# intelligent-machine-learning/tfplus

Hardware: AMD Instinct MI355X
Metric: lookups+GroupAdam-applies/sec and HBM GB/s, 1M int64 ids x dim32 (higher is better)
Workload: dtype f32; 1 GPU; configs[1]: 50M-key KvVariable x dim32 per GPU, 1000000 ids/batch per GPU Zipf(1.2), lookup + sparse GroupAdam apply; keys=50000000, dim=32, batch=1000000, global_batch=1000000, parallelism=single GPU

## Files before the change

tfplus_amd/csrc/kv_device.h:

```cpp
#pragma once

constexpr long long EMPTY_KEY = (long long)0x8000000000000000ULL;
constexpr unsigned FLAG_BLACK = 1u;
constexpr unsigned FLAG_UNDER = 2u;
constexpr unsigned FLAG_DIRTY = 4u;
constexpr float CUTOFF = 1.0e-20f;
constexpr unsigned FLAG_FREE = 8u;
constexpr unsigned ROW_TOMB = 0xFFFFFFFFu;
constexpr unsigned ROW_FILTERED = 0x80000000u;
constexpr unsigned ROW_MASK = 0x7FFFFFFFu;
constexpr unsigned HEAD_BIT = 0x80000000u;
constexpr unsigned BASE_MASK = 0x3FFFFFFFu;
constexpr int RANK_SHIFT = 21;
constexpr unsigned SLOT_MASK = (1u << RANK_SHIFT) - 1u;
constexpr int LCOLD = 16;
constexpr int HC = 128;
constexpr unsigned EP_TAG = 0x40000000u;
constexpr unsigned NEW_BIT = 0x80000000u;
constexpr unsigned HINT_NEW = 0xFFFFFFFFu;
constexpr int HC2 = 512;

constexpr int TB = 256;
#ifndef KV_TBT
#define KV_TBT 512
// ... 198 lines not shown
  return r;
}

__device__ __forceinline__ void init_rule_rows(const TableDev& t, long long key, const float** ia, const float** ib, int D) {
  const unsigned long long h = pick64((unsigned long long)key ^ (t.seed * 0x9E3779B97F4A7C15ULL));
  *ia = t.init_table + (size_t)((unsigned)h % t.init_rows) * D;
  *ib = t.init_table + (size_t)((unsigned)(h >> 32) % t.init_rows) * D;
}
__device__ __forceinline__ void init_rule_rows(const TableDev& t, long long key, const float** ia, const float** ib) {
  init_rule_rows(t, key, ia, ib, t.dim);
}
__device__ __forceinline__ bool init_row_coop(const TableDev& t, long long key, float* dst,
                                              int lane, int lanes) {
  const float *a, *b;
  init_rule_rows(t, key, &a, &b);
  bool big = false;
  for (int e = lane; e < t.dim; e += lanes) {
    float v = (a[e] + b[e]) * 0.5f;
    dst[e] = v;
    big |= fabsf(v) >= CUTOFF;
  }
  return big;
}

__device__ __forceinline__ unsigned part_of(long long key, int pshift) {
  return pshift >= 64 ? 0u : (unsigned)(mix64((unsigned long long)key) >> pshift);
}

__device__ __forceinline__ void lds_barrier() { asm volatile("s_waitcnt lgkmcnt(0)\n\ts_barrier" ::: "memory"); }

template <int NW, bool LDSONLY = false>
__device__ __forceinline__ unsigned block_excl_scan(unsigned v, unsigned* wtot, unsigned* total) {
  const int lane = threadIdx.x & 63, wv = threadIdx.x >> 6;
  unsigned incl = v;
#pragma unroll
  for (int o = 1; o < 64; o <<= 1) {
    const unsigned x = __shfl_up(incl, o);
    if (lane >= o) incl += x;
  }
  if (LDSONLY) lds_barrier(); else __syncthreads();
  if (lane == 63) wtot[wv] = incl;
  if (LDSONLY) lds_barrier(); else __syncthreads();
  unsigned base = 0, tot = 0;
#pragma unroll
  for (int i = 0; i < NW; ++i) {
    const unsigned x = wtot[i];
    if (i < wv) base += x;
    tot += x;
  }
  *total = tot;
  return base + incl - v;
}

template <typename IdT>
__device__ __forceinline__ long long load_id(const IdT* ids, size_t i) {
  return (long long)ids[i];
}
struct IdCount { long long id, count; };
template <>
__device__ __forceinline__ long long load_id<IdCount>(const IdCount* ids, size_t i) { return ids[i].id; }

#ifdef KV_FASTM_CONST
#define KV_FASTM(a) (KV_FASTM_CONST != 0)
#else
#define KV_FASTM(a) ((a).fast != 0)
#endif
__device__ __forceinline__ float kv_sqrt(float x, bool fast) { return fast ? __builtin_amdgcn_sqrtf(x) : sqrtf(x); }
__device__ __forceinline__ float kv_div(float x, float y, bool fast) { return fast ? x * __builtin_amdgcn_rcpf(y) : x / y; }

__device__ __forceinline__ unsigned slot_find_or_insert(const TableDev& t, long long key,
                                                       unsigned day, bool* inserted) {
  unsigned r = table_find_or_insert(t, key, inserted);
  if (r == 0) return 0;
  unsigned* fp = freq_ptr(t, r);
  if (*inserted) {
    *fp = 1u;
  } else {
    unsigned lo = (*fp & 0xFFFFu) + 1u;
    if (lo > 65535u) lo = 65535u;
    *fp = (day << 16) | lo;
  }
  return r;
}

template <int V>
__device__ __forceinline__ void ldv(const float* p, float (&o)[V]) {
  if (V == 4) {
    const float4 t4 = *reinterpret_cast<const float4*>(p);
    o[0] = t4.x; o[1 % V] = t4.y; o[2 % V] = t4.z; o[3 % V] = t4.w;
  } else {
    o[0] = p[0];
  }
}
template <int V>
__device__ __forceinline__ void ldv_stream(const float* p, float (&o)[V]) {
#pragma unroll
  for (int c = 0; c < V; ++c) o[c] = __builtin_nontemporal_load(p + c);
}
template <int V>
__device__ __forceinline__ void stv(float* p, const float (&o)[V]) {
  if (V == 4) {
    *reinterpret_cast<float4*>(p) = make_float4(o[0], o[1 % V], o[2 % V], o[3 % V]);
  } else {
    p[0] = o[0];
  }
}
// ... 461 lines not shown
```

tfplus_amd/csrc/kv_fused.h:

```cpp
#pragma once

__device__ __forceinline__ unsigned tile_insert(const TableDev& t, long long key) {
  Entry* slot;
  unsigned long long stored;
  unsigned long long p = 0;
  const bool sentinel = key == EMPTY_KEY;
  if (sentinel) { slot = &t.entries[t.mask + 1]; stored = 0ull; }
  else { stored = (unsigned long long)key; p = mix64((unsigned long long)key) & t.mask; slot = &t.entries[p]; }
  for (;;) {
    const Entry e = load_entry(slot);
    if ((unsigned long long)e.key == stored && !(sentinel && e.key == EMPTY_KEY)) {
      if (e.row == ROW_TOMB) {
        if (atomicCAS(&slot->row, ROW_TOMB, 0u) == ROW_TOMB) break;
        return NEW_BIT;
      }
      if (e.row == 0u || e.hint == HINT_NEW) return NEW_BIT | e.row;
      return e.row;
    }
    if (e.key == EMPTY_KEY) {
      const unsigned long long old = atomicCAS(reinterpret_cast<unsigned long long*>(&slot->key),
                                               (unsigned long long)EMPTY_KEY, stored);
      if (old == (unsigned long long)EMPTY_KEY) break;
      if (old == stored) return NEW_BIT;
      if (sentinel) continue;
// ... 406 lines not shown
      unsigned before = 0;
      for (int wv = 0; wv < TBT / 64; ++wv) {
        if (wave == wv && valid) {
          before = run[e];
          if (rw == 0u) run[e] = (unsigned short)(before + cnt);
        }
        lds_barrier();
      }
      myrank[k] = valid ? before + rw : 0u;
    }
  }
#pragma unroll
  for (int k = 0; k < IPT; ++k) {
    if (tslot[k] == 0xFFFFFFFFu || sm.lcnt[tslot[k]] <= 1u) continue;
    const unsigned pre = sm.escan[sm.lpos[tslot[k]]];
    sm.mr[(pre & ES_POS) + myrank[k]] = (unsigned)(k * TBT + tid) | ((pre >> ES_NSH) << 11) | (myrank[k] == 0u ? 0x80000000u : 0u);
  }
  if (has_counts) {
    lds_barrier();
    for (unsigned e = tid; e <= (unsigned)TILE; e += TBT) sm.hist[e] = 0;
    lds_barrier();
#pragma unroll
    for (int k = 0; k < IPT; ++k)
      if (tslot[k] != 0xFFFFFFFFu) atomicAdd(&sm.hist[sm.lpos[tslot[k]]], creg[k]);
    lds_barrier();
#pragma unroll
    for (int k = 0; k < IPT; ++k) {
      if (wpos[k] == 0xFFFFFFFFu) continue;
      const unsigned f = sm.hist[wpos[k]];
      w.ent_a[(size_t)tile * TILE + wpos[k]] = wcnt[k] | ((f > 65535u ? 65535u : f) << 16);
    }
  }
  lds_barrier();
  {
    unsigned* dst = w.mrow + (size_t)tile * TILE;
    for (int j = tid; j < TILE; j += TBT) dst[j] = sm.mr[j];
  }
  KV_STAMP(4);
  if constexpr (GATHER) {
#pragma unroll
    for (int k = 0; k < IPT; ++k) rr[k] = tslot[k] != 0xFFFFFFFFu ? sm.lrow[tslot[k]] : 0u;
    if (__builtin_expect(pf == 1.2345678e-38f, 0)) sm.wtot[0] = 1u;
    output_rows();
  }
  KV_STAMP(5);
}

template <typename IdT, int VQ, bool GATHER, bool NOTABLE = false>
__global__ void __launch_bounds__(TBT, 4) k_ltile(TableDev t, WsDev w, const IdT* __restrict__ ids,
                                              const int* __restrict__ counts, long long n, int det, float* __restrict__ out) {
  ltile_body<IdT, VQ, GATHER, NOTABLE>(t, w, ids, counts, n, det, out);
}

template <int T, int NW>
__device__ __forceinline__ unsigned seg_directory_t(const WsDev& w, unsigned p, unsigned short* tpre,
                                                    unsigned short* tstart, unsigned* wtot, unsigned* pbase) {
  const unsigned NT = w.ntiles;
  unsigned run0 = 0, pb = 0;
  for (unsigned tb = 0; tb < NT; tb += T) {
    const unsigned t = tb + threadIdx.x;
    unsigned len = 0, s0 = 0;
    if (t < NT) {
      const unsigned* c0 = w.toff + (size_t)t * (w.P + 1) + p;
      const unsigned a = c0[0], b = c0[1];
      s0 = a & 0xFFFFu;
      len = (b & 0xFFFFu) - s0;
      tstart[t] = (unsigned short)s0;
    }
    unsigned tot;
    const unsigned ex = block_excl_scan<NW>(len, wtot, &tot);
    unsigned tot2;
    block_excl_scan<NW>(s0, wtot, &tot2);
    if (t < NT) tpre[t] = (unsigned short)min(run0 + ex, 65535u);
    run0 += tot;
    pb += tot2;
  }
  __syncthreads();
  *pbase = pb;
  return run0;
}
__device__ __forceinline__ void part2_body(const WsDev& w, const PartArgs& a) {
  constexpr int HSK = 1024;
  constexpr int UCAPK = HSK - TBK;
  constexpr int EB = 8;
  __shared__ long long hkey[HSK + 1];
  __shared__ unsigned hval[HSK + 1];
  __shared__ unsigned hrow[HSK + 1];
  __shared__ unsigned short lnew[UCAPK + 8];
  __shared__ unsigned short ulist[UCAPK + 8];
  __shared__ unsigned lnu, lsent, lnnew, lkeys;
  __shared__ unsigned wtot[8];
  extern __shared__ __attribute__((aligned(16))) char smem_raw[];
  unsigned short* tpre = reinterpret_cast<unsigned short*>(smem_raw);
  unsigned short* tstart = tpre + w.ntiles;

  const int tid = threadIdx.x;
  const unsigned p = xcd_partition(blockIdx.x, w.P);
  const unsigned NT = w.ntiles;
  const int D = a.tv.dim;
  KV_STAMPP(0);
  unsigned pbase;
  const unsigned E = seg_directory_t<TBK, TBK / 64>(w, p, tpre, tstart, wtot, &pbase);
  if (E == 0) return;
  __shared__ unsigned stkR[24], stkr[24];
  __shared__ int sp;
  if (tid == 0) { stkR[0] = 1; stkr[0] = 0; sp = 1; lkeys = 0; }
  __syncthreads();
  if (E > 65535u) {
    if (tid == 0) raise_error(a.tv, 2u);
    return;
  }
  while (sp > 0) {
    const unsigned R = stkR[sp - 1], round = stkr[sp - 1];
    __syncthreads();
    if (tid == 0) --sp;
    for (int s = tid; s <= HSK; s += TBK) { hkey[s] = EMPTY_KEY; hval[s] = 0; hrow[s] = 0; }
    if (tid == 0) { lnu = 0; lsent = 0; lnnew = 0; }
    __syncthreads();
    for (unsigned x0 = 0; x0 < E; x0 += EB * TBK) {
      unsigned ge[EB];
      long long key[EB];
      unsigned ea[EB], rw[EB];
#pragma unroll
      for (int k = 0; k < EB; ++k) {
        const unsigned x = x0 + k * TBK + tid;
        ge[k] = x < E ? (unsigned)seg_entry(tpre, tstart, NT, x) : 0xFFFFFFFFu;
      }
#pragma unroll
      for (int k = 0; k < EB; ++k) {
        key[k] = 0; ea[k] = 0; rw[k] = 0;
        if (ge[k] != 0xFFFFFFFFu) { key[k] = w.ent_key[ge[k]]; ea[k] = w.ent_a[ge[k]]; rw[k] = w.ent_b[ge[k]]; }
      }
#pragma unroll
      for (int k = 0; k < EB; ++k) {
        if (ge[k] == 0xFFFFFFFFu || !in_round(key[k], R, round)) continue;
        if (lnu >= (unsigned)UCAPK) continue;
        bool first;
        const unsigned h = lds_key_slot<HSK>(hkey, &lsent, key[k], true, &first);
        if (first) {
          const unsigned u = atomicAdd(&lnu, 1u);
          if (u < (unsigned)UCAPK) ulist[u] = (unsigned short)h;
        }
        atomicAdd(&hval[h], ea[k] >> 16);
        atomicMax(&hrow[h], rw[k]);
      }
    }
    __syncthreads();
    if (lnu >= (unsigned)UCAPK) {
      __syncthreads();
      if (tid == 0) {
        if (sp + 2 <= 24) {
          stkR[sp] = 2 * R; stkr[sp] = round; ++sp;
          stkR[sp] = 2 * R; stkr[sp] = round + R; ++sp;
        } else {
          raise_error(a.tv, 2u);
        }
      }
      __syncthreads();
      continue;
    }
    KV_STAMPP(1);
    const unsigned nu = lnu;
    if (tid == 0) lkeys += nu;

    constexpr int PERU = (UCAPK + TBK - 1) / TBK;
    {
      unsigned sl[PERU], r[PERU];
      bool isnew[PERU];
      uint2 m[PERU];
#pragma unroll
      for (int k = 0; k < PERU; ++k) {
        const unsigned u = tid * PERU + k;
        sl[k] = 0xFFFFFFFFu; r[k] = 0; isnew[k] = false; m[k] = make_uint2(0u, (unsigned)FLAG_DIRTY);
        if (u < nu) {
          sl[k] = ulist[u];
          const unsigned rw = hrow[sl[k]];
          r[k] = rw & ROW_MASK; isnew[k] = (rw & NEW_BIT) != 0u;
          if (r[k] != 0u && !isnew[k]) m[k] = load_freq_flags(a.tv, r[k]);
        }
      }
#pragma unroll
      for (int k = 0; k < PERU; ++k) {
        if (sl[k] == 0xFFFFFFFFu) continue;
        const unsigned s = sl[k];
        const long long key = (s == HSK) ? EMPTY_KEY : hkey[s];
        if (__builtin_expect(isnew[k], 0)) {
          Entry* e = table_entry_of(a.tv, key);
          if (e) {
            if (r[k] == 0u) { const unsigned er = load_entry(e).row; r[k] = er != ROW_TOMB ? er : 0u; }
            e->hint = 0u;
          }
          hrow[s] = r[k] | NEW_BIT;
        }
        if (r[k] == 0u) continue;
        RowMeta* mp = meta_ptr(a.tv, r[k]);
        if (isnew[k]) { mp->key = key; mp->delta = 0; mp->stamp = 0; }
        mark_delta(a.tv, r[k]);
        const unsigned cnt = a.count_once ? 1u : hval[s];
        mp->freq = (a.day << 16) | freq_add_sat(m[k].x, cnt);
        if (isnew[k]) mp->flags = (unsigned char)FLAG_DIRTY;
        if (m[k].y & FLAG_DIRTY) lnew[atomicAdd(&lnnew, 1u)] = (unsigned short)(s | (isnew[k] ? 0x8000u : 0u));
      }
    }
    __syncthreads();
    KV_STAMPP(2);

    {
      const int lane8 = tid & 7;
      const unsigned nn = lnnew;
      const unsigned npad = (nn + 7u) & ~7u;
      for (unsigned j = tid >> 3; j < npad; j += TBK / 8) {
        const bool live = j < nn;
        const unsigned sv = live ? lnew[j] : 0u;
        const unsigned s = sv & 0x7FFFu;
        const bool isnew = (sv & 0x8000u) != 0;
        const long long key = (s == HSK) ? EMPTY_KEY : hkey[s];
        const unsigned r = live ? (hrow[s] & ROW_MASK) : 0u;
        float* row = row_ptr(a.tv, r);
        bool big = false;
        if (live && r != 0) {
          if (isnew) big = init_row_coop(a.tv, key, row, lane8, 8);
          else
            for (int e = lane8; e < D; e += 8) big |= fabsf(row[e]) >= CUTOFF;
        }
        const unsigned long long mb = __ballot(big);
        const bool any = ((mb >> ((tid & 63) & ~7)) & 0xFFull) != 0;
        if (live && r != 0 && lane8 == 0) {
          unsigned char* fp = flags_ptr(a.tv, r);
          const unsigned black = isnew ? 0u : (*fp & FLAG_BLACK);
          *fp = (unsigned char)(black ? (FLAG_BLACK | FLAG_UNDER) : (any ? 0u : FLAG_UNDER));
        }
      }
    }
    __syncthreads();
    KV_STAMPP(3);
  }
  if (tid == 0) atomicAdd(&w.ctr[5], lkeys);
}
__global__ void __launch_bounds__(TBK, 4) k_part2(WsDev w, PartArgs a) { part2_body(w, a); }

constexpr int TBC = TBT;
static_assert(TBC == TBT, "k_ltsum: the tile pass and the tile sums share one block");
template <int V, int LPR, int K, bool FROM_LDS = false>
__device__ __forceinline__ void tsum_body(const WsDev& w, const float* __restrict__ grad, int D, unsigned tile,
                                          const unsigned* mrow_l = nullptr, unsigned mc_l = 0u) {
  constexpr int G = 64 / LPR;
  constexpr int RB = (8 / K) > 0 ? (8 / K) : 1;
  constexpr int RS = G * RB;
  constexpr int NWC = TBC / 64;
  constexpr int RF = K * V * LPR;
  __shared__ float lfs[2][NWC][RF];
  __shared__ unsigned lmeta[NWC][2];
  const unsigned mc = FROM_LDS ? mc_l : w.mcount[tile];
  const unsigned nm = mc & 0xFFFFu;
  if (nm == 0u) return;
  const unsigned* const mrow_g = w.mrow + (size_t)tile * TILE;
  const float* g0 = grad + (size_t)tile * TILE * D;
  const float* g0s = w.grad_self + (size_t)tile * TILE * D;
  const unsigned tbase = tile * (unsigned)TILE;
  float* ep = w.epart + (size_t)tile * (TILE / 2) * D;
  const int wl = threadIdx.x & 63, lane = wl % LPR, g = wl / LPR, wv = threadIdx.x >> 6;
  int eoff[K];
  bool evalid[K];
#pragma unroll
  for (int k = 0; k < K; ++k) { const int e0 = (lane + k * LPR) * V; evalid[k] = e0 < D; eoff[k] = evalid[k] ? e0 : 0; }
  auto store_row = [&](unsigned slot, const float (&v)[K][V]) {
    float* dst = ep + (size_t)slot * D;
#pragma unroll
    for (int k = 0; k < K; ++k)
      if (evalid[k]) stv<V>(dst + eoff[k], v[k]);
  };
  const unsigned steps = (nm + (unsigned)(NWC * RS) - 1u) / (unsigned)(NWC * RS);
  const unsigned r0 = (unsigned)wv * steps * RS, r1 = min(nm, r0 + steps * RS);
  float carry[K][V];
#pragma unroll
  for (int k = 0; k < K; ++k)
#pragma unroll
    for (int cc = 0; cc < V; ++cc) carry[k][cc] = 0.f;
  bool seen = false;
  unsigned last_slot = 0;
  unsigned mw[RB], mn[RB];
  auto ldm = [&](unsigned rbase, unsigned (&m)[RB]) {
#pragma unroll
    for (int i = 0; i < RB; ++i) {
      const unsigned r = rbase + g * RB + i, rc = r < r1 ? r : (r0 < nm ? r0 : 0u);
      if constexpr (FROM_LDS) m[i] = mrow_l[rc]; else m[i] = mrow_g[rc];
    }
  };
// ... 212 lines not shown
```

tfplus_amd/csrc/kv_papply.h:

```cpp
#pragma once

#ifndef KV_PA_WAVES
#define KV_PA_WAVES 4
#endif
#ifndef KV_PA_HOTRB
#define KV_PA_HOTRB 8
#endif
#ifndef KV_PA_RC
#define KV_PA_RC 4
#endif
template <int TBP> struct PaShape { static constexpr int HSK = TBP >= 512 ? 2048 : 1024, LSRC = TBP >= 512 ? 2048 : 1536; };

template <int OPT, int V, int LPR, int K, int TBP, int FM = -1>
__device__ __forceinline__ void papply_body(const WsDev& w, const PartArgs& a, const int mode_) {
  constexpr bool UQ = FM == PA_UNIQUE, DN = FM == PA_DEDUP_NUM, DD = FM == PA_DEDUP || DN;
  const int mode = FM >= 0 ? (DN ? (int)PA_DEDUP : FM) : (mode_ & 0xFF);
  constexpr int HSK = PaShape<TBP>::HSK;
  constexpr int PA_LSRC = PaShape<TBP>::LSRC;
  constexpr int UCAPK = (HSK - TBP) < 1023 ? (HSK - TBP) : 1023;
  constexpr int EB = 8;
  constexpr int G = 64 / LPR;
  constexpr int RB = (KV_PA_HOTRB / K) > 0 ? (KV_PA_HOTRB / K) : 1;
  constexpr int NW = TBP / 64;
  __shared__ long long hkey[HSK + 1];
  __shared__ unsigned hval[DD ? 1 : HSK + 1];
  __shared__ unsigned hrow[HSK + 1];
  __shared__ unsigned hhint[(UQ || DD) ? 1 : HSK + 1];
  __shared__ unsigned hocc[HSK + 1];
  __shared__ unsigned short hcn[HSK + 1];
  __shared__ unsigned short ulist[UCAPK + 8];
  __shared__ unsigned short kord[UCAPK + 8];
  __shared__ unsigned lsrc[PA_LSRC];
  __shared__ unsigned lnu, lsent, lnext, lkeys, lbase;
  __shared__ unsigned rh[MAXW], rbase[MAXW];
  __shared__ unsigned wtot[8];
  __shared__ unsigned stkR[24], stkr[24];
  __shared__ int sp;
  extern __shared__ __attribute__((aligned(16))) char smem_raw[];
  unsigned short* tpre = reinterpret_cast<unsigned short*>(smem_raw);
  unsigned short* tstart = tpre + w.ntiles;

  const int tid = threadIdx.x;
  const unsigned p = xcd_partition(blockIdx.x, w.P);
  const unsigned NT = w.ntiles;
  const int D = a.tv.dim;
  const unsigned errflag = *reinterpret_cast<volatile unsigned*>(&a.tv.counters[1]);
  KV_STAMPP(0);
  unsigned pbase = 0;
  const unsigned E = seg_directory_t<TBP, NW>(w, p, tpre, tstart, wtot, &pbase);
  KV_STAMPP(5);
  if (E == 0) return;
  if (tid == 0) { sp = 0; lkeys = 0; }
  __syncthreads();
  if (E > 65535u) {
    if (tid == 0) raise_error(a.tv, 2u);
    return;
  }
  const bool in_lds = E <= (unsigned)PA_LSRC;
  unsigned* const gsrc = w.order + pbase;
  auto src_at = [&](unsigned i) -> unsigned {
    return in_lds ? lsrc[i] : __hip_atomic_load(gsrc + i, __ATOMIC_RELAXED, __HIP_MEMORY_SCOPE_AGENT);
  };

  auto do_round = [&](const unsigned R, const unsigned round) -> bool {
    __syncthreads();
    for (int s = tid; s <= HSK; s += TBP) {
      hkey[s] = EMPTY_KEY; hrow[s] = 0; hocc[s] = 0;
      if constexpr (!DD) hval[s] = 0;
      if constexpr (!UQ && !DD) hhint[s] = 0;
    }
    if (tid == 0) { lnu = 0; lsent = 0; lnext = 0; }
    __syncthreads();
    unsigned csrc[EB];
    unsigned short cslot[EB];
    bool cin[EB];
    const bool cached = (R == 1 && E <= (unsigned)(EB * TBP));
    for (unsigned x0 = 0; x0 < E; x0 += EB * TBP) {
      unsigned ge[EB];
      long long key[EB];
      unsigned ea[EB], rw[EB], hi[EB], sr[EB];
#pragma unroll
      for (int k = 0; k < EB; ++k) {
        const unsigned x = x0 + k * TBP + tid;
        ge[k] = x < E ? (unsigned)seg_entry(tpre, tstart, NT, x) : 0xFFFFFFFFu;
      }
#pragma unroll
      for (int k = 0; k < EB; ++k) {
        key[k] = 0; ea[k] = 0; rw[k] = 0; hi[k] = 0; sr[k] = 0;
        if (ge[k] != 0xFFFFFFFFu) {
          key[k] = w.ent_key[ge[k]]; ea[k] = w.ent_a[ge[k]]; rw[k] = w.ent_b[ge[k]]; hi[k] = w.ent_base[ge[k]];
          if (cached) sr[k] = w.ent_rec[ge[k]];
        }
      }
#pragma unroll
      for (int k = 0; k < EB; ++k) {
        if (x0 == 0) { csrc[k] = sr[k]; cslot[k] = 0; cin[k] = false; }
        if (ge[k] == 0xFFFFFFFFu || !in_round(key[k], R, round)) continue;
        if (lnu >= (unsigned)UCAPK) continue;
        bool first;
        const unsigned h = lds_key_slot<HSK>(hkey, &lsent, key[k], true, &first);
        if (first) {
          const unsigned u = atomicAdd(&lnu, 1u);
          if (u < (unsigned)UCAPK) ulist[u] = (unsigned short)h;
        }
        if constexpr (UQ) atomicAdd(&hval[h], a.sparse_unique ? (ea[k] & 0xFFFFu) : (ea[k] >> 16));
        else if constexpr (!DD) { if (mode == PA_LOOKUP) atomicAdd(&hval[h], ea[k] >> 16); }
        atomicAdd(&hocc[h], 1u);
        atomicMax(&hrow[h], rw[k]);
        if constexpr (!UQ && !DD) { if (hi[k]) atomicMax(&hhint[h], hi[k]); }
        if (x0 == 0) { cslot[k] = (unsigned short)h; cin[k] = true; }
      }
    }
    __syncthreads();
    if (lnu >= (unsigned)UCAPK) return true;
    KV_STAMPP(1);
    const unsigned nu = lnu;
    const unsigned lkeys_before = lkeys;
    __syncthreads();
    if (tid == 0) {
      lkeys += nu;
      if ((UQ && !a.sparse_unique) || DN) lbase = atomicAdd(&w.ctr[0], nu);
    }

    constexpr int PERU = (UCAPK + TBP - 1) / TBP;
    unsigned nhot, ncold;
    {
      unsigned kcnt[PERU];
      unsigned sum = 0, ch = 0, hh = 0;
#pragma unroll
      for (int q = 0; q < PERU; ++q) {
        const unsigned u = tid * PERU + q;
        kcnt[q] = u < nu ? hocc[ulist[u]] : 0u;
        sum += kcnt[q];
        if (u < nu) {
          if (kcnt[q] == 1u) ch += 1u;
          else if (kcnt[q] == 2u) ch += 1u << 10;
          else if (kcnt[q] <= (unsigned)LCOLD) ch += 1u << 20;
          else hh += 1u;
        }
      }
      unsigned tot, chtot, htot;
      unsigned run = block_excl_scan<NW>(sum, wtot, &tot);
      unsigned chrun = block_excl_scan<NW>(ch, wtot, &chtot);
      unsigned hrn = block_excl_scan<NW>(hh, wtot, &htot);
      const unsigned t1 = chtot & 1023u, t2 = (chtot >> 10) & 1023u;
      nhot = htot; ncold = nu - htot;
#pragma unroll
      for (int q = 0; q < PERU; ++q) {
        const unsigned u = tid * PERU + q;
        if (u < nu) {
          const unsigned s = ulist[u];
          unsigned rank;
          if (kcnt[q] == 1u) { rank = nhot + (chrun & 1023u); chrun += 1u; }
          else if (kcnt[q] == 2u) { rank = nhot + t1 + ((chrun >> 10) & 1023u); chrun += 1u << 10; }
          else if (kcnt[q] <= (unsigned)LCOLD) { rank = nhot + t1 + t2 + (chrun >> 20); chrun += 1u << 20; }
          else { rank = hrn; hrn += 1u; }
          kord[rank] = (unsigned short)s;
          hocc[s] = run; run += kcnt[q];
          hcn[s] = (unsigned short)kcnt[q];
          if (UQ) {
            const unsigned num = a.sparse_unique ? pbase + lkeys_before + u : lbase + u;
            hrow[s] = num;
            a.out_keys[num] = (s == (unsigned)HSK) ? EMPTY_KEY : hkey[s];
            if (a.sparse_unique) a.out_counts[num] = (int)hval[s];
            else if (a.out_counts) a.out_counts[num] = (int)(hval[s] > 65535u ? 65535u : hval[s]);
          }
          if (DN) {
            const unsigned num = lbase + u;
            hrow[s] = num;
            a.out_keys[num] = (s == (unsigned)HSK) ? EMPTY_KEY : hkey[s];
          }
        }
      }
    }
    __syncthreads();
    if (UQ && a.route_world > 0) {
      if (tid < MAXW) rh[tid] = 0;
      __syncthreads();
      unsigned rd[PERU], rr[PERU];
#pragma unroll
      for (int q = 0; q < PERU; ++q) {
        const unsigned u = tid * PERU + q;
        rd[q] = 0xFFFFFFFFu; rr[q] = 0;
        if (u < nu) {
          const unsigned s = ulist[u];
          const long long key = (s == (unsigned)HSK) ? EMPTY_KEY : hkey[s];
          rd[q] = owner_rank(key, a.route_world, a.route_rule);
          rr[q] = atomicAdd(&rh[rd[q]], 1u);
        }
      }
      __syncthreads();
      if (tid < a.route_world) rbase[tid] = rh[tid] ? atomicAdd(&a.route_gcount[tid], rh[tid]) : 0u;
      __syncthreads();
#pragma unroll
      for (int q = 0; q < PERU; ++q) {
        const unsigned u = tid * PERU + q;
        if (u < nu) {
          const unsigned s = ulist[u];
          const unsigned num = hrow[s];
          const unsigned at = rbase[rd[q]] + rr[q];
          if (at < a.route_C) {
            const size_t slot = (size_t)rd[q] * (a.route_C + 1) + 1 + at;
            a.route_seg[2 * slot] = (s == (unsigned)HSK) ? EMPTY_KEY : hkey[s];
            a.route_seg[2 * slot + 1] = (long long)(int)hval[s];
            a.route_slot_of[num] = (int)slot;
          } else {
            a.route_slot_of[num] = 0;
            atomicExch(a.route_overflow, 1u);
          }
        }
      }
    }

    {
      constexpr bool numbers = UQ || DN;
      auto file = [&](unsigned pos, unsigned src) { if (in_lds) lsrc[pos] = src; else gsrc[pos] = src; };
      if (a.det) {
        const int wave = tid >> 6, wl = tid & 63;
        for (unsigned x0 = 0; x0 < E; x0 += TBP) {
          const unsigned x = x0 + tid;
          bool valid = x < E;
          size_t ge = 0;
          unsigned h = 0xFFFFFFFFu;
          if (valid) {
            ge = seg_entry(tpre, tstart, NT, x);
            const long long key = w.ent_key[ge];
            valid = in_round(key, R, round);
            if (valid) { bool first; h = lds_key_slot<HSK>(hkey, &lsent, key, false, &first); }
          }
          unsigned within = 0;
          for (int j = 0; j < 63; ++j) {
            const unsigned hj = __shfl(h, j);
            if (j < wl && hj == h) within += 1u;
          }
          unsigned pos = 0;
          for (int wv = 0; wv < NW; ++wv) {
            if (wave == wv && valid) { pos = hocc[h] + within; atomicAdd(&hocc[h], 1u); }
            __syncthreads();
          }
          if (valid) { file(pos, w.ent_rec[ge]); if (numbers) w.ent_b[ge] = hrow[h]; }
        }
      } else if (cached) {
#pragma unroll
        for (int k = 0; k < EB; ++k)
          if (cin[k]) {
            file(atomicAdd(&hocc[cslot[k]], 1u), csrc[k]);
            if (numbers) w.ent_b[seg_entry(tpre, tstart, NT, (unsigned)(k * TBP + tid))] = hrow[cslot[k]];
          }
      } else {
        for (unsigned x = tid; x < E; x += TBP) {
          const size_t ge = seg_entry(tpre, tstart, NT, x);
          const long long key = w.ent_key[ge];
          const unsigned src = w.ent_rec[ge];
          if (!in_round(key, R, round)) continue;
          bool first;
          const unsigned h = lds_key_slot<HSK>(hkey, &lsent, key, false, &first);
          file(atomicAdd(&hocc[h], 1u), src);
          if (numbers) w.ent_b[ge] = hrow[h];
        }
      }
    }
    if (!in_lds) __threadfence_block();
    __syncthreads();
    KV_STAMPP(2);

    unsigned tid2 = threadIdx.x;
    asm volatile("" : "+v"(tid2));
    const int wl = (int)(tid2 & 63u), lane = wl % LPR, g = wl / LPR;
    const float* const gbase = a.grad;
    const float* const ebase = a.epart;
    const float* const gself = w.grad_self;
    int eoff[K];
    bool evalid[K];
  #pragma unroll
    for (int k = 0; k < K; ++k) { const int e0 = (lane + k * LPR) * V; evalid[k] = e0 < D; eoff[k] = evalid[k] ? e0 : 0; }
    const LeanCtx lc = lean_ctx<OPT>(a);
    constexpr int NS0 = slot0_blocks(OPT);

    const unsigned nbatch = (ncold + (unsigned)G - 1u) / (unsigned)G;
    const unsigned nitems = nhot + nbatch;
    KV_STAMPPV(6, E); KV_STAMPPV(7, nu); KV_STAMPPV(8, nhot);
    if (UQ) return false;
#ifdef KV_STAMPS
    unsigned long long st_t0 = wall_clock64(), st_hot = 0, st_cold = 0, st_nh = 0, st_nc = 0;
#endif
    for (;;) {
#ifdef KV_STAMPS
      const unsigned long long st_a = wall_clock64();
#endif
      unsigned it = 0;
      if (wl == 0) it = atomicAdd(&lnext, 1u);
      it = (unsigned)__builtin_amdgcn_readfirstlane((int)it);
      if (it >= nitems) break;
      int eo[K];
#pragma unroll
      for (int k = 0; k < K; ++k) { eo[k] = eoff[k]; asm volatile("" : "+v"(eo[k])); }
      int lane_i = lane;
      asm volatile("" : "+v"(lane_i));
      auto load_row = [&](unsigned pos, float (&dst)[K][V]) {
        const float* base = (pos & EP_TAG) ? ebase : (pos - w.self_lo < w.self_len) ? gself : gbase;
        const float* src = base + (size_t)(pos & ~EP_TAG) * D;
// ... 173 lines not shown
            if (oflags & FLAG_DIRTY) {
              const unsigned black = nk ? 0u : (oflags & FLAG_BLACK);
              nfl = black ? (FLAG_BLACK | FLAG_UNDER) : (any ? 0u : (unsigned)FLAG_UNDER);
            }
            if (lane == 0) {
              RowMeta* mp = meta_ptr(a.tv, row);
              if (nk) {
                RowMeta nm; nm.key = key; nm.freq = nf; nm.flags = (unsigned char)nfl;
                nm.delta = a.tv.track_delta ? (unsigned char)DELTA_TRAIN : 0; nm.stamp = 0;
                *mp = nm;
              } else {
                mp->freq = nf;
                if (nfl != oflags) mp->flags = (unsigned char)nfl;
                if (a.tv.track_delta) mp->delta |= (unsigned char)DELTA_TRAIN;
              }
            }
            vm.x = nf; vm.y = (vm.y & ~0xFFu) | nfl;
          }
        } else if (nk) {
          const unsigned nfl = any ? 0u : (unsigned)FLAG_UNDER;
          if (lane == 0) {
            RowMeta nm; nm.key = key; nm.freq = 1u; nm.flags = (unsigned char)nfl;
            nm.delta = 0; nm.stamp = 0;
            *meta_ptr(a.tv, row) = nm;
          }
          vm.x = 1u; vm.y = nfl;
          vnew = true;
        }
      }

      const bool fin_live = live && errflag == 0u;
      const uint4 ra = make_uint4((unsigned)key, (unsigned)((unsigned long long)key >> 32), row | (vnew ? NEW_BIT : 0u), hint);
      const bool general = key_update<OPT, V, LPR, K>(a, lc, row, hint, vnew, fin_live, lane_i, D, gv, vm, mir, pre);
      if (!lc.fast || __ballot(general) != 0ull)
        finish_key<MODE_APPLY, OPT, V, LPR, K>(a, ra, general, hint_loaded && general, m0, gv, lane_i, &pre, have_x && general,
                                               have_s && general);
#ifdef KV_STAMPS
      {
        const unsigned long long now = wall_clock64();
        if (is_hot) { st_hot += now - st_a; ++st_nh; } else { st_cold += now - st_a; ++st_nc; }
      }
#endif
    }
#ifdef KV_STAMPS
    if (wl == 0) {
      unsigned long long* d = w.dbg + (size_t)(8192 + blockIdx.x * NW + (tid >> 6)) * 16;
      d[0] = st_t0; d[1] = wall_clock64(); d[2] = st_hot; d[3] = st_cold; d[4] = st_nh; d[5] = st_nc;
    }
#endif
    __syncthreads();
    KV_STAMPP(3);
    return false;
  };
  if (do_round(1u, 0u)) {
    __syncthreads();
    if (tid == 0) { stkR[0] = 2; stkr[0] = 0; stkR[1] = 2; stkr[1] = 1; sp = 2; }
    __syncthreads();
    while (sp > 0) {
      const unsigned R = stkR[sp - 1], round = stkr[sp - 1];
      __syncthreads();
      if (tid == 0) --sp;
      const bool ovf = do_round(R, round);
      __syncthreads();
      if (ovf && tid == 0) {
        if (sp + 2 <= 24) {
          stkR[sp] = 2 * R; stkr[sp] = round; ++sp;
          stkR[sp] = 2 * R; stkr[sp] = round + R; ++sp;
        } else {
          raise_error(a.tv, 2u);
        }
      }
      __syncthreads();
    }
  }
  if (tid == 0 && mode != PA_NONE && !DD) atomicAdd(&w.ctr[5], lkeys);
}

__device__ __forceinline__ void papply_route_tail(const PartArgs& a, const int mode_, const unsigned nblocks) {
  if ((mode_ & 0xFF) != PA_UNIQUE || a.route_world <= 0 || a.route_need == nullptr) return;
  __shared__ unsigned rt_last, rt_tot, rt_max;
  __syncthreads();
  if (threadIdx.x == 0) {
    rt_last = __hip_atomic_fetch_add(&a.route_gcount[MAXW], 1u, __ATOMIC_RELAXED, __HIP_MEMORY_SCOPE_AGENT) == nblocks - 1u ? 1u : 0u;
    rt_tot = 0u; rt_max = 0u;
  }
  __syncthreads();
  if (!rt_last) return;
  const int d = (int)threadIdx.x;
  if (d < a.route_world) {
    const unsigned c = __hip_atomic_load(&a.route_gcount[d], __ATOMIC_RELAXED, __HIP_MEMORY_SCOPE_AGENT);
    __hip_atomic_store(&a.route_gcount[d], 0u, __ATOMIC_RELAXED, __HIP_MEMORY_SCOPE_AGENT);
    a.route_seg[2 * (size_t)d * (a.route_C + 1)] = c < a.route_C ? c : a.route_C;
    a.route_seg[2 * (size_t)d * (a.route_C + 1) + 1] = 0;
    atomicMax(&rt_max, c);
    atomicAdd(&rt_tot, c);
  }
  __syncthreads();
  if (d == 0) {
    __hip_atomic_store(&a.route_gcount[MAXW], 0u, __ATOMIC_RELAXED, __HIP_MEMORY_SCOPE_AGENT);
    *a.route_need = rt_max;
    if (a.route_uhint) __hip_atomic_store(a.route_uhint, rt_tot, __ATOMIC_RELAXED, __HIP_MEMORY_SCOPE_SYSTEM);
  }
}

template <int OPT, int V, int LPR, int K, int TBP>
__global__ void __launch_bounds__(TBP, KV_PA_WAVES) k_papply(WsDev w, PartArgs a, int mode) {
  papply_body<OPT, V, LPR, K, TBP>(w, a, mode);
}

template <int TBP>
__global__ void __launch_bounds__(TBP, KV_PA_WAVES) k_papply_uniq(WsDev w, PartArgs a, int mode) {
  papply_body<OPT_ADAM_V4, 4, 1, 1, TBP, PA_UNIQUE>(w, a, mode);
  papply_route_tail(a, mode, gridDim.x);
}
#ifndef KV_PD_WAVES
// ... 49 lines not shown
```

Baseline: 7.840 billion ids/s (each id: 1 embedding lookup + 1 fused GroupAdam-V4 apply).

## Prefetch first segment entries during directory scan and pack prefix scans into 64-bit

The partition kernels now load each thread's first few entries of its own tile while building the segment directory. Hash clearing overlaps with those loads, and the first round inserts from registers, skipping the binary-search gather when no tile has more entries than fit in the prefetch. The directory scan and the three hot/cold/count scans are each packed into a single 64-bit block scan, which cuts barriers and LDS round trips. This adds register pressure, more template complexity and a separate path for leftover entries. It also depends on the bit-packing bounds holding.

Measured after the change: 7.549 billion ids/s (each id: 1 embedding lookup + 1 fused GroupAdam-V4 apply). 3.7% lower.

```diff
diff --git a/tfplus_amd/csrc/kv_device.h b/tfplus_amd/csrc/kv_device.h
--- a/tfplus_amd/csrc/kv_device.h
+++ b/tfplus_amd/csrc/kv_device.h
@@ -274,6 +274,35 @@
   return base + incl - v;
 }
 
+__device__ __forceinline__ unsigned long long wave_incl_scan64(unsigned long long v) {
+  const int lane = threadIdx.x & 63;
+  unsigned long long incl = v;
+#pragma unroll
+  for (int o = 1; o < 64; o <<= 1) {
+    const unsigned long long x = __shfl_up(incl, o);
+    if (lane >= o) incl += x;
+  }
+  return incl;
+}
+template <int NW, bool LDSONLY = false>
+__device__ __forceinline__ unsigned long long block_excl_scan64(unsigned long long v, unsigned long long* wtot,
+                                                                unsigned long long* total) {
+  const int lane = threadIdx.x & 63, wv = threadIdx.x >> 6;
+  const unsigned long long incl = wave_incl_scan64(v);
+  if (LDSONLY) lds_barrier(); else __syncthreads();
+  if (lane == 63) wtot[wv] = incl;
+  if (LDSONLY) lds_barrier(); else __syncthreads();
+  unsigned long long base = 0, tot = 0;
+#pragma unroll
+  for (int i = 0; i < NW; ++i) {
+    const unsigned long long x = wtot[i];
+    if (i < wv) base += x;
+    tot += x;
+  }
+  *total = tot;
+  return base + incl - v;
+}
+
 template <typename IdT>
 __device__ __forceinline__ long long load_id(const IdT* ids, size_t i) {
   return (long long)ids[i];
diff --git a/tfplus_amd/csrc/kv_fused.h b/tfplus_amd/csrc/kv_fused.h
--- a/tfplus_amd/csrc/kv_fused.h
+++ b/tfplus_amd/csrc/kv_fused.h
@@ -482,32 +482,61 @@
   ltile_body<IdT, VQ, GATHER, NOTABLE>(t, w, ids, counts, n, det, out);
 }
 
-template <int T, int NW>
+template <int T, int NW, int EBF, class Fetch, class UnderLoads>
 __device__ __forceinline__ unsigned seg_directory_t(const WsDev& w, unsigned p, unsigned short* tpre,
-                                                    unsigned short* tstart, unsigned* wtot, unsigned* pbase) {
+                                                    unsigned short* tstart, unsigned long long* wtot, unsigned* pbase,
+                                                    bool* rest, Fetch&& fetch, UnderLoads&& under_loads) {
   const unsigned NT = w.ntiles;
+  const int lane = threadIdx.x & 63, wv = threadIdx.x >> 6;
   unsigned run0 = 0, pb = 0;
+  bool rs = false;
   for (unsigned tb = 0; tb < NT; tb += T) {
     const unsigned t = tb + threadIdx.x;
-    unsigned len = 0, s0 = 0;
+    unsigned a = 0, b = 0;
     if (t < NT) {
       const unsigned* c0 = w.toff + (size_t)t * (w.P + 1) + p;
-      const unsigned a = c0[0], b = c0[1];
-      s0 = a & 0xFFFFu;
-      len = (b & 0xFFFFu) - s0;
-      tstart[t] = (unsigned short)s0;
-    }
-    unsigned tot;
-    const unsigned ex = block_excl_scan<NW>(len, wtot, &tot);
-    unsigned tot2;
-    block_excl_scan<NW>(s0, wtot, &tot2);
+      a = c0[0]; b = c0[1];
+    }
+    if (tb == 0) under_loads();
+    const unsigned s0 = a & 0xFFFFu;
+    const unsigned len = (b & 0xFFFFu) - s0;
+    if (tb == 0) {
+      fetch(t, s0, len);
+      if (len != 0xFFFFFFFEu) KV_STAMPP(9);
+    }
+    if (t < NT) tstart[t] = (unsigned short)s0;
+    const unsigned long long v = ((unsigned long long)len << 32) | s0;
+    const unsigned long long incl = wave_incl_scan64(v);
+    const bool wrest = __ballot(tb == 0 ? len > (unsigned)EBF : len > 0u) != 0ull;
+    if (tb != 0) lds_barrier();
+    if (lane == 63) wtot[wv] = incl | (wrest ? 1ull << 63 : 0ull);
+    lds_barrier();
+    unsigned long long base = 0, tot = 0;
+#pragma unroll
+    for (int i = 0; i < NW; ++i) {
+      const unsigned long long x = wtot[i];
+      rs |= (x >> 63) != 0ull;
+      if (i < wv) base += x & ~(1ull << 63);
+      tot += x & ~(1ull << 63);
+    }
+    const unsigned ex = (unsigned)((base + incl - v) >> 32);
     if (t < NT) tpre[t] = (unsigned short)min(run0 + ex, 65535u);
-    run0 += tot;
-    pb += tot2;
-  }
-  __syncthreads();
-  *pbase = pb;
-  return run0;
+    run0 += (unsigned)(tot >> 32);
+    pb += (unsigned)tot;
+  }
+  *pbase = (unsigned)__builtin_amdgcn_readfirstlane((int)pb);
+  *rest = __builtin_amdgcn_readfirstlane((int)rs) != 0;
+  return (unsigned)__builtin_amdgcn_readfirstlane((int)run0);
+}
+__device__ __forceinline__ size_t seg_entry_at(const unsigned short* tpre, const unsigned short* tstart, unsigned NT,
+                                               unsigned x, unsigned* tile, unsigned* j) {
+  unsigned lo = 0, hi = NT;
+  while (hi - lo > 1) {
+    const unsigned mid = (lo + hi) >> 1;
+    if (tpre[mid] <= x) lo = mid; else hi = mid;
+  }
+  *tile = lo; *j = x - tpre[lo];
+  return (size_t)lo * TILE + tstart[lo] + (x - tpre[lo]);
 }
 __device__ __forceinline__ void part2_body(const WsDev& w, const PartArgs& a) {
   constexpr int HSK = 1024;
@@ -519,7 +548,7 @@
   __shared__ unsigned short lnew[UCAPK + 8];
   __shared__ unsigned short ulist[UCAPK + 8];
   __shared__ unsigned lnu, lsent, lnnew, lkeys;
-  __shared__ unsigned wtot[8];
+  __shared__ unsigned long long wtot[8];
   extern __shared__ __attribute__((aligned(16))) char smem_raw[];
   unsigned short* tpre = reinterpret_cast<unsigned short*>(smem_raw);
   unsigned short* tstart = tpre + w.ntiles;
@@ -529,50 +558,86 @@
   const unsigned NT = w.ntiles;
   const int D = a.tv.dim;
   KV_STAMPP(0);
-  unsigned pbase;
-  const unsigned E = seg_directory_t<TBK, TBK / 64>(w, p, tpre, tstart, wtot, &pbase);
-  if (E == 0) return;
   __shared__ unsigned stkR[24], stkr[24];
   __shared__ int sp;
-  if (tid == 0) { stkR[0] = 1; stkr[0] = 0; sp = 1; lkeys = 0; }
-  __syncthreads();
+  auto clear_hash = [&]() {
+    for (int s = tid; s <= HSK; s += TBK) { hkey[s] = EMPTY_KEY; hval[s] = 0; hrow[s] = 0; }
+    if (tid == 0) { lnu = 0; lsent = 0; lnnew = 0; }
+  };
+  auto insert = [&](long long key, unsigned ea, unsigned rw) {
+    if (lnu >= (unsigned)UCAPK) return;
+    bool first;
+    const unsigned h = lds_key_slot<HSK>(hkey, &lsent, key, true, &first);
+    if (first) {
+      const unsigned u = atomicAdd(&lnu, 1u);
+      if (u < (unsigned)UCAPK) ulist[u] = (unsigned short)h;
+    }
+    atomicAdd(&hval[h], ea >> 16);
+    atomicMax(&hrow[h], rw);
+  };
+  constexpr int EBF = 4;
+  long long fkey[EBF];
+  unsigned fea[EBF], frw[EBF], flen = 0;
+  unsigned pbase;
+  bool rest;
+  const unsigned E = seg_directory_t<TBK, TBK / 64, EBF>(
+      w, p, tpre, tstart, wtot, &pbase, &rest,
+      [&](unsigned t, unsigned s0, unsigned len) {
+        flen = len;
+        const unsigned g0 = t * (unsigned)TILE + s0;
+#pragma unroll
+        for (int k = 0; k < EBF; ++k) {
+          fkey[k] = 0; fea[k] = 0; frw[k] = 0;
+          if ((unsigned)k < len) { fkey[k] = w.ent_key[g0 + k]; fea[k] = w.ent_a[g0 + k]; frw[k] = w.ent_b[g0 + k]; }
+        }
+      },
+      [&]() {
+        clear_hash();
+        if (tid == 0) { stkR[0] = 1; stkr[0] = 0; sp = 1; lkeys = 0; }
+      });
+  if (E == 0) return;
   if (E > 65535u) {
     if (tid == 0) raise_error(a.tv, 2u);
     return;
   }
-  while (sp > 0) {
-    const unsigned R = stkR[sp - 1], round = stkr[sp - 1];
+  auto do_round = [&](auto firstc, const unsigned R, const unsigned round) {
+    constexpr bool first_round = decltype(firstc)::value;
     __syncthreads();
     if (tid == 0) --sp;
-    for (int s = tid; s <= HSK; s += TBK) { hkey[s] = EMPTY_KEY; hval[s] = 0; hrow[s] = 0; }
-    if (tid == 0) { lnu = 0; lsent = 0; lnnew = 0; }
-    __syncthreads();
-    for (unsigned x0 = 0; x0 < E; x0 += EB * TBK) {
-      unsigned ge[EB];
-      long long key[EB];
-      unsigned ea[EB], rw[EB];
-#pragma unroll
-      for (int k = 0; k < EB; ++k) {
-        const unsigned x = x0 + k * TBK + tid;
-        ge[k] = x < E ? (unsigned)seg_entry(tpre, tstart, NT, x) : 0xFFFFFFFFu;
-      }
-#pragma unroll
-      for (int k = 0; k < EB; ++k) {
-        key[k] = 0; ea[k] = 0; rw[k] = 0;
-        if (ge[k] != 0xFFFFFFFFu) { key[k] = w.ent_key[ge[k]]; ea[k] = w.ent_a[ge[k]]; rw[k] = w.ent_b[ge[k]]; }
-      }
-#pragma unroll
-      for (int k = 0; k < EB; ++k) {
-        if (ge[k] == 0xFFFFFFFFu || !in_round(key[k], R, round)) continue;
-        if (lnu >= (unsigned)UCAPK) continue;
-        bool first;
-        const unsigned h = lds_key_slot<HSK>(hkey, &lsent, key[k], true, &first);
-        if (first) {
-          const unsigned u = atomicAdd(&lnu, 1u);
-          if (u < (unsigned)UCAPK) ulist[u] = (unsigned short)h;
-        }
-        atomicAdd(&hval[h], ea[k] >> 16);
-        atomicMax(&hrow[h], rw[k]);
+    if constexpr (!first_round) {
+      clear_hash();
+      __syncthreads();
+    }
+    if constexpr (first_round) {
+#pragma unroll
+      for (int k = 0; k < EBF; ++k)
+        if ((unsigned)k < flen) insert(fkey[k], fea[k], frw[k]);
+    }
+    if (!first_round || rest) {
+      for (unsigned x0 = 0; x0 < E; x0 += EB * TBK) {
+        unsigned ge[EB];
+        long long key[EB];
+        unsigned ea[EB], rw[EB];
+#pragma unroll
+        for (int k = 0; k < EB; ++k) {
+          const unsigned x = x0 + k * TBK + tid;
+          ge[k] = 0xFFFFFFFFu;
+          if (x < E) {
+            unsigned tile, j;
+            const unsigned g = (unsigned)seg_entry_at(tpre, tstart, NT, x, &tile, &j);
+            if (!(first_round && tile < (unsigned)TBK && j < (unsigned)EBF)) ge[k] = g;
+          }
+        }
+#pragma unroll
+        for (int k = 0; k < EB; ++k) {
+          key[k] = 0; ea[k] = 0; rw[k] = 0;
+          if (ge[k] != 0xFFFFFFFFu) { key[k] = w.ent_key[ge[k]]; ea[k] = w.ent_a[ge[k]]; rw[k] = w.ent_b[ge[k]]; }
+        }
+#pragma unroll
+        for (int k = 0; k < EB; ++k) {
+          if (ge[k] == 0xFFFFFFFFu || !in_round(key[k], R, round)) continue;
+          insert(key[k], ea[k], rw[k]);
+        }
       }
     }
     __syncthreads();
@@ -587,7 +652,7 @@
         }
       }
       __syncthreads();
-      continue;
+      return;
     }
     KV_STAMPP(1);
     const unsigned nu = lnu;
@@ -664,6 +729,11 @@
     }
     __syncthreads();
     KV_STAMPP(3);
+  };
+  do_round(std::true_type{}, 1u, 0u);
+  while (sp > 0) {
+    const unsigned R = stkR[sp - 1], round = stkr[sp - 1];
+    do_round(std::false_type{}, R, round);
   }
   if (tid == 0) atomicAdd(&w.ctr[5], lkeys);
 }
diff --git a/tfplus_amd/csrc/kv_papply.h b/tfplus_amd/csrc/kv_papply.h
--- a/tfplus_amd/csrc/kv_papply.h
+++ b/tfplus_amd/csrc/kv_papply.h
@@ -33,7 +33,7 @@
   __shared__ unsigned lsrc[PA_LSRC];
   __shared__ unsigned lnu, lsent, lnext, lkeys, lbase;
   __shared__ unsigned rh[MAXW], rbase[MAXW];
-  __shared__ unsigned wtot[8];
+  __shared__ unsigned long long wtot[8];
   __shared__ unsigned stkR[24], stkr[24];
   __shared__ int sp;
   extern __shared__ __attribute__((aligned(16))) char smem_raw[];
@@ -46,12 +46,39 @@
   const int D = a.tv.dim;
   const unsigned errflag = *reinterpret_cast<volatile unsigned*>(&a.tv.counters[1]);
   KV_STAMPP(0);
+  auto clear_hash = [&]() {
+    for (int s = tid; s <= HSK; s += TBP) {
+      hkey[s] = EMPTY_KEY; hrow[s] = 0; hocc[s] = 0;
+      if constexpr (!DD) hval[s] = 0;
+      if constexpr (!UQ && !DD) hhint[s] = 0;
+    }
+    if (tid == 0) { lnu = 0; lsent = 0; lnext = 0; }
+  };
+  long long fkey[EB];
+  unsigned fea[EB], frw[EB], fhi[EB], fsr[EB], flen = 0;
   unsigned pbase = 0;
-  const unsigned E = seg_directory_t<TBP, NW>(w, p, tpre, tstart, wtot, &pbase);
+  bool rest;
+  const unsigned E = seg_directory_t<TBP, NW, EB>(
+      w, p, tpre, tstart, wtot, &pbase, &rest,
+      [&](unsigned t, unsigned s0, unsigned len) {
+        flen = len;
+        const unsigned g0 = t * (unsigned)TILE + s0;
+#pragma unroll
+        for (int k = 0; k < EB; ++k) {
+          fkey[k] = 0; fea[k] = 0; frw[k] = 0; fhi[k] = 0; fsr[k] = 0;
+          if ((unsigned)k < len) {
+            fkey[k] = w.ent_key[g0 + k]; fea[k] = w.ent_a[g0 + k]; frw[k] = w.ent_b[g0 + k];
+            if constexpr (!UQ && !DD) fhi[k] = w.ent_base[g0 + k];
+            fsr[k] = w.ent_rec[g0 + k];
+          }
+        }
+      },
+      [&]() {
+        clear_hash();
+        if (tid == 0) { sp = 0; lkeys = 0; }
+      });
   KV_STAMPP(5);
   if (E == 0) return;
-  if (tid == 0) { sp = 0; lkeys = 0; }
-  __syncthreads();
   if (E > 65535u) {
     if (tid == 0) raise_error(a.tv, 2u);
     return;
@@ -62,53 +89,81 @@
     return in_lds ? lsrc[i] : __hip_atomic_load(gsrc + i, __ATOMIC_RELAXED, __HIP_MEMORY_SCOPE_AGENT);
   };
 
-  auto do_round = [&](const unsigned R, const unsigned round) -> bool {
-    __syncthreads();
-    for (int s = tid; s <= HSK; s += TBP) {
-      hkey[s] = EMPTY_KEY; hrow[s] = 0; hocc[s] = 0;
-      if constexpr (!DD) hval[s] = 0;
-      if constexpr (!UQ && !DD) hhint[s] = 0;
-    }
-    if (tid == 0) { lnu = 0; lsent = 0; lnext = 0; }
-    __syncthreads();
+  auto do_round = [&](auto firstc, const unsigned R, const unsigned round) -> bool {
+    constexpr bool FIRST = decltype(firstc)::value;
+    if constexpr (!FIRST) {
+      __syncthreads();
+      clear_hash();
+      __syncthreads();
+    }
     unsigned csrc[EB];
     unsigned short cslot[EB];
     bool cin[EB];
-    const bool cached = (R == 1 && E <= (unsigned)(EB * TBP));
-    for (unsigned x0 = 0; x0 < E; x0 += EB * TBP) {
-      unsigned ge[EB];
-      long long key[EB];
-      unsigned ea[EB], rw[EB], hi[EB], sr[EB];
+    unsigned gsrc_[EB];
+    unsigned short gslot[EB];
+    bool gin[EB];
+    const bool cached = FIRST && (!rest || E <= (unsigned)(EB * TBP));
+    auto insert = [&](long long key, unsigned ea, unsigned rw, unsigned hi) -> unsigned {
+      bool first;
+      const unsigned h = lds_key_slot<HSK>(hkey, &lsent, key, true, &first);
+      if (first) {
+        const unsigned u = atomicAdd(&lnu, 1u);
+        if (u < (unsigned)UCAPK) ulist[u] = (unsigned short)h;
+      }
+      if constexpr (UQ) atomicAdd(&hval[h], a.sparse_unique ? (ea & 0xFFFFu) : (ea >> 16));
+      else if constexpr (!DD) { if (mode == PA_LOOKUP) atomicAdd(&hval[h], ea >> 16); }
+      atomicAdd(&hocc[h], 1u);
+      atomicMax(&hrow[h], rw);
+      if constexpr (!UQ && !DD) { if (hi) atomicMax(&hhint[h], hi); }
+      return h;
+    };
+    if constexpr (FIRST) {
+      if (fkey[0] != 0x7FFFFFFFFFFFFFF1ll) KV_STAMPP(12);
 #pragma unroll
       for (int k = 0; k < EB; ++k) {
-        const unsigned x = x0 + k * TBP + tid;
-        ge[k] = x < E ? (unsigned)seg_entry(tpre, tstart, NT, x) : 0xFFFFFFFFu;
-      }
-#pragma unroll
-      for (int k = 0; k < EB; ++k) {
-        key[k] = 0; ea[k] = 0; rw[k] = 0; hi[k] = 0; sr[k] = 0;
-        if (ge[k] != 0xFFFFFFFFu) {
-          key[k] = w.ent_key[ge[k]]; ea[k] = w.ent_a[ge[k]]; rw[k] = w.ent_b[ge[k]]; hi[k] = w.ent_base[ge[k]];
-          if (cached) sr[k] = w.ent_rec[ge[k]];
-        }
-      }
-#pragma unroll
-      for (int k = 0; k < EB; ++k) {
-        if (x0 == 0) { csrc[k] = sr[k]; cslot[k] = 0; cin[k] = false; }
-        if (ge[k] == 0xFFFFFFFFu || !in_round(key[k], R, round)) continue;
-        if (lnu >= (unsigned)UCAPK) continue;
-        bool first;
-        const unsigned h = lds_key_slot<HSK>(hkey, &lsent, key[k], true, &first);
-        if (first) {
-          const unsigned u = atomicAdd(&lnu, 1u);
-          if (u < (unsigned)UCAPK) ulist[u] = (unsigned short)h;
-        }
-        if constexpr (UQ) atomicAdd(&hval[h], a.sparse_unique ? (ea[k] & 0xFFFFu) : (ea[k] >> 16));
-        else if constexpr (!DD) { if (mode == PA_LOOKUP) atomicAdd(&hval[h], ea[k] >> 16); }
-        atomicAdd(&hocc[h], 1u);
-        atomicMax(&hrow[h], rw[k]);
-        if constexpr (!UQ && !DD) { if (hi[k]) atomicMax(&hhint[h], hi[k]); }
-        if (x0 == 0) { cslot[k] = (unsigned short)h; cin[k] = true; }
+        csrc[k] = fsr[k]; cslot[k] = 0; cin[k] = false;
+        if ((unsigned)k >= flen || lnu >= (unsigned)UCAPK) continue;
+        cslot[k] = (unsigned short)insert(fkey[k], fea[k], frw[k], fhi[k]);
+        cin[k] = true;
+      }
+    }
+    if constexpr (FIRST) {
+#pragma unroll
+      for (int k = 0; k < EB; ++k) gin[k] = false;
+    }
+    if (!FIRST || rest) {
+      if (FIRST) lds_barrier();
+      for (unsigned x0 = 0; x0 < E; x0 += EB * TBP) {
+        unsigned ge[EB];
+        long long key[EB];
+        unsigned ea[EB], rw[EB], hi[EB], sr[EB];
+#pragma unroll
+        for (int k = 0; k < EB; ++k) {
+          const unsigned x = x0 + k * TBP + tid;
+          ge[k] = 0xFFFFFFFFu;
+          if (x < E) {
+            unsigned tile, j;
+            const unsigned g = (unsigned)seg_entry_at(tpre, tstart, NT, x, &tile, &j);
+            if (!(FIRST && tile < (unsigned)TBP && j < (unsigned)EB)) ge[k] = g;
+          }
+        }
+#pragma unroll
+        for (int k = 0; k < EB; ++k) {
+          key[k] = 0; ea[k] = 0; rw[k] = 0; hi[k] = 0; sr[k] = 0;
+          if (ge[k] != 0xFFFFFFFFu) {
+            key[k] = w.ent_key[ge[k]]; ea[k] = w.ent_a[ge[k]]; rw[k] = w.ent_b[ge[k]];
+            if constexpr (!UQ && !DD) hi[k] = w.ent_base[ge[k]];
+            if (cached) sr[k] = w.ent_rec[ge[k]];
+          }
+        }
+#pragma unroll
+        for (int k = 0; k < EB; ++k) {
+          if (FIRST && x0 == 0) { gsrc_[k] = sr[k]; gslot[k] = 0; gin[k] = false; }
+          if (ge[k] == 0xFFFFFFFFu || !in_round(key[k], R, round)) continue;
+          if (lnu >= (unsigned)UCAPK) continue;
+          const unsigned h = insert(key[k], ea[k], rw[k], hi[k]);
+          if (FIRST && x0 == 0) { gslot[k] = (unsigned short)h; gin[k] = true; }
+        }
       }
     }
     __syncthreads();
@@ -139,10 +194,11 @@
           else hh += 1u;
         }
       }
-      unsigned tot, chtot, htot;
-      unsigned run = block_excl_scan<NW>(sum, wtot, &tot);
-      unsigned chrun = block_excl_scan<NW>(ch, wtot, &chtot);
-      unsigned hrn = block_excl_scan<NW>(hh, wtot, &htot);
+      unsigned long long ptot;
+      const unsigned long long prun =
+          block_excl_scan64<NW>((unsigned long long)ch | ((unsigned long long)hh << 30) | ((unsigned long long)sum << 40), wtot, &ptot);
+      unsigned run = (unsigned)(prun >> 40), chrun = (unsigned)prun & 0x3FFFFFFFu, hrn = (unsigned)(prun >> 30) & 1023u;
+      const unsigned chtot = (unsigned)ptot & 0x3FFFFFFFu, htot = (unsigned)(ptot >> 30) & 1023u;
       const unsigned t1 = chtot & 1023u, t2 = (chtot >> 10) & 1023u;
       nhot = htot; ncold = nu - htot;
 #pragma unroll
@@ -174,6 +230,7 @@
       }
     }
     __syncthreads();
+    KV_STAMPP(13);
     if (UQ && a.route_world > 0) {
       if (tid < MAXW) rh[tid] = 0;
       __syncthreads();
@@ -245,8 +302,16 @@
         for (int k = 0; k < EB; ++k)
           if (cin[k]) {
             file(atomicAdd(&hocc[cslot[k]], 1u), csrc[k]);
-            if (numbers) w.ent_b[seg_entry(tpre, tstart, NT, (unsigned)(k * TBP + tid))] = hrow[cslot[k]];
-          }
+            if (numbers) w.ent_b[(unsigned)tid * (unsigned)TILE + tstart[tid] + k] = hrow[cslot[k]];
+          }
+        if (rest) {
+#pragma unroll
+          for (int k = 0; k < EB; ++k)
+            if (gin[k]) {
+              file(atomicAdd(&hocc[gslot[k]], 1u), gsrc_[k]);
+              if (numbers) w.ent_b[seg_entry(tpre, tstart, NT, (unsigned)(k * TBP + tid))] = hrow[gslot[k]];
+            }
+        }
       } else {
         for (unsigned x = tid; x < E; x += TBP) {
           const size_t ge = seg_entry(tpre, tstart, NT, x);
@@ -526,7 +591,7 @@
     KV_STAMPP(3);
     return false;
   };
-  if (do_round(1u, 0u)) {
+  if (do_round(std::true_type{}, 1u, 0u)) {
     __syncthreads();
     if (tid == 0) { stkR[0] = 2; stkr[0] = 0; stkR[1] = 2; stkr[1] = 1; sp = 2; }
     __syncthreads();
@@ -534,7 +599,7 @@
       const unsigned R = stkR[sp - 1], round = stkr[sp - 1];
       __syncthreads();
       if (tid == 0) --sp;
-      const bool ovf = do_round(R, round);
+      const bool ovf = do_round(std::false_type{}, R, round);
       __syncthreads();
       if (ovf && tid == 0) {
         if (sp + 2 <= 24) {
```
